# castorini/dhr

Measured on AMD Instinct MI355X. Metric: queries/sec (exact top-1000, brute-force dense-hybrid GIP retrieval), higher is better.
Workload: dtype i8 (bound GEMM: gated AND ungated columns int8 x int8 -> int32 on the matrix cores, every gated rounding upward, the ungated quantisation error paid by the filter margin) + f64-accumulated f16 x f32 exact rescoring of the survivors -- the returned scores are the exact scores rounded once, identical

## Files before the change

### dhr_amd/_lib.py

```python
from __future__ import annotations

import ctypes as C
import os

import numpy as np

from . import _build

DHR_OK = 0
ERR_INVALID, ERR_UNSUPPORTED, ERR_HIP, ERR_INTERNAL, ERR_NOMEM, ERR_PEER = -1, -2, -3, -4, -5, -6
ABI_INDEX_DESC, ABI_QUERY_BATCH, ABI_SEARCH_STATS, ABI_FILE_INFO, ABI_HOST_SHARD = 0, 1, 2, 3, 4
IDX_NONE, IDX_U8, IDX_I8, IDX_I16 = 0, 1, 2, 3
VAL_F16, VAL_F32 = 0, 1
MEM_HOST, MEM_DEVICE = 0, 1
LEX_RAW, LEX_DENSIFY, LEX_AGG_FULL, LEX_AGG_SEMI = 0, 1, 2, 3
PARAM_CAND_CAP, PARAM_FIRST_ROWS, PARAM_PROFILE, PARAM_MAX_GROWTH, PARAM_SAMPLE_PERIOD, PARAM_GEMM_VARIANT, PARAM_MAIN_CHUNKS, PARAM_PROGRESSIVE_THR, PARAM_AUX_CUS, PARAM_GEMM_EXCLUSIVE, PARAM_OVERLAP_AUX, PARAM_SAMPLE_SHARE, PARAM_ASYNC_CONTROLLER, PARAM_LIST_STRIDE = 1, 2, 3, 4, 5, 6, 7, 8, 9, 10, 11, 12, 13, 14
OPT_DENSE_I8, OPT_GATED_I8 = 1, 2
COMM_TRANSPORT, COMM_WORLD, COMM_RANK, COMM_DEVICE = 0, 1, 2, 3
INFO_DENSE_I8, INFO_I8_SCALE, INFO_I8_ROW_ERR, INFO_I8_ROW_NORM, INFO_ROW_NORM_MAX, INFO_TILE_BYTES, INFO_GATED_I8, INFO_GEMM_KERNEL = 1, 2, 3, 4, 5, 6, 7, 8

EXPORTS = ["dhr_version", "dhr_abi_sizes", "dhr_abi_size", "dhr_debug_fail_alloc", "dhr_set_option", "dhr_index_get_info", "dhr_last_error", "dhr_index_create", "dhr_index_destroy", "dhr_index_set_param",
           "dhr_index_device_bytes", "dhr_search", "dhr_score_rows", "dhr_merge_topk", "dhr_merge_topk_host", "dhr_merge_topk_lists", "dhr_merge_topk_lists_host",
           "dhr_get_stats", "dhr_debug_bound_scores", "dhr_debug_query_margins", "dhr_debug_gemm_time", "dhr_debug_seq_to_tile", "dhr_debug_sharded_repairs", "dhr_search_sample_rank", "dhr_search_union_rank", "dhr_search_begin",
           "dhr_search_finish", "dhr_search_mid_ranks", "dhr_search_mid", "dhr_search_pre_ranks", "dhr_search_pre", "dhr_search_begin_rest", "dhr_search_rerank", "dhr_comm_unique_id", "dhr_comm_create", "dhr_comm_wrap", "dhr_comm_create_callback", "dhr_comm_destroy", "dhr_comm_info", "dhr_comm_abort", "dhr_search_sharded", "dhr_search_sharded_local", "dhr_search_sharded_host", "dhr_pq_create", "dhr_pq_destroy", "dhr_pq_device_bytes", "dhr_pq_search", "dhr_pq_adc_scores", "dhr_pq_last_scan", "dhr_index_save", "dhr_index_file_info", "dhr_index_load", "dhr_densify", "dhr_pq_train", "dhr_pq_encode", "dhr_pq_decode", "dhr_pq_train_nbits", "dhr_pq_encode_nbits", "dhr_pq_decode_nbits", "dhr_write_trec", "dhr_format_float", "dhr_lexical_head", "dhr_aggregate", "dhr_gip_scores_workspace", "dhr_gip_scores", "dhr_gip_scores_backward", "dhr_densify_backward", "dhr_lexical_head_train_workspace", "dhr_lexical_head_train", "dhr_lexical_head_backward", "dhr_maxsim_scores", "dhr_maxsim_scores_backward", "dhr_aggregate_train", "dhr_aggregate_backward", "dhr_term_weight_head",
           "dhr_term_weight_head_backward", "dhr_lexical_proj_workspace", "dhr_lexical_proj_head", "dhr_lexical_proj_train_workspace",
           "dhr_lexical_proj_train", "dhr_lexical_proj_backward", "dhr_train_loss_workspace", "dhr_train_loss"]


class DhrError(RuntimeError):

    def __init__(self, msg, status=None):
        super().__init__(msg)
        self.status = status


class IndexDesc(C.Structure):
    _fields_ = [("device", C.c_int32), ("mem_kind", C.c_int32), ("n_rows", C.c_int64), ("d_dlr", C.c_int32),
                ("d_cls", C.c_int32), ("value", C.c_void_p), ("ld_value", C.c_int64), ("index", C.c_void_p),
                ("index_dtype", C.c_int32), ("idx_buckets", C.c_int32), ("ld_index", C.c_int64),
                ("row_offset", C.c_int64)]


class QueryBatch(C.Structure):
    _fields_ = [("n_queries", C.c_int32), ("mem_kind", C.c_int32), ("value", C.c_void_p), ("value_dtype", C.c_int32),
                ("index_dtype", C.c_int32), ("ld_value", C.c_int64), ("index", C.c_void_p), ("ld_index", C.c_int64)]

# ... 166 lines not shown
    lib.dhr_comm_abort.argtypes = [C.c_void_p]
    lib.dhr_comm_abort.restype = None
    lib.dhr_comm_info.argtypes = [C.c_void_p, C.c_int32]
    lib.dhr_search_sharded.argtypes = [C.c_void_p, C.c_void_p, C.POINTER(QueryBatch), C.c_int32, C.c_void_p, C.c_void_p, C.c_int32, C.c_void_p]
    lib.dhr_search_sharded_local.argtypes = [C.POINTER(C.c_void_p), C.c_int32, C.POINTER(QueryBatch), C.c_int32, C.c_void_p, C.c_void_p, C.c_int32, C.c_void_p]
    lib.dhr_pq_create.argtypes = [C.c_int32, C.c_int32, C.c_int64, C.c_int32, C.c_int32, C.c_int32, C.c_void_p, C.c_void_p, C.c_int64, C.POINTER(C.c_void_p)]
    lib.dhr_pq_destroy.argtypes = [C.c_void_p]
    lib.dhr_pq_destroy.restype = None
    lib.dhr_pq_device_bytes.argtypes = [C.c_void_p]
    lib.dhr_pq_device_bytes.restype = C.c_int64
    lib.dhr_pq_search.argtypes = [C.c_void_p, C.POINTER(QueryBatch), C.c_int32, C.c_void_p, C.c_void_p, C.c_int32, C.c_void_p]
    lib.dhr_pq_adc_scores.argtypes = [C.c_void_p, C.POINTER(QueryBatch), C.c_int64, C.c_int64, C.c_void_p, C.c_void_p]
    lib.dhr_pq_last_scan.argtypes = [C.c_void_p, C.POINTER(C.c_double), C.POINTER(C.c_double)]
    lib.dhr_get_stats.argtypes = [C.c_void_p, C.POINTER(SearchStats)]
    lib.dhr_set_option.argtypes = [C.c_int32, C.c_int64]
    lib.dhr_index_get_info.argtypes = [C.c_void_p, C.c_int32, C.POINTER(C.c_double)]
    lib.dhr_debug_bound_scores.argtypes = [C.c_void_p, C.POINTER(QueryBatch), C.c_int64, C.c_int64, C.c_void_p, C.c_void_p]
    lib.dhr_debug_query_margins.argtypes = [C.c_void_p, C.POINTER(QueryBatch), C.c_void_p, C.c_void_p]
    lib.dhr_debug_gemm_time.argtypes = [C.c_void_p, C.POINTER(QueryBatch), C.c_int32, C.POINTER(C.c_double),
                                        C.POINTER(C.c_double), C.c_void_p]
    if hasattr(lib, "dhr_debug_seq_to_tile"):
        lib.dhr_debug_seq_to_tile.argtypes = [C.c_int64, C.c_int32, C.c_int32, C.c_int64, C.c_int64, C.c_int64, C.POINTER(C.c_int64)]
        lib.dhr_debug_seq_to_tile.restype = None
    lib.dhr_search_sample_rank.argtypes = [C.c_void_p, C.c_int32]
    lib.dhr_search_sample_rank.restype = C.c_int32
    lib.dhr_search_union_rank.argtypes = [C.c_void_p, C.c_int32]
    lib.dhr_search_union_rank.restype = C.c_int32
    lib.dhr_search_begin.argtypes = [C.c_void_p, C.POINTER(QueryBatch), C.c_int32, C.c_void_p, C.c_void_p]
    lib.dhr_search_finish.argtypes = [C.c_void_p, C.c_void_p, C.c_void_p, C.c_void_p, C.c_void_p, C.c_int32, C.c_void_p]
    lib.dhr_search_mid_ranks.argtypes = [C.c_void_p, C.c_int32, C.POINTER(C.c_int32), C.POINTER(C.c_int32)]
    lib.dhr_search_mid_ranks.restype = C.c_int32
    lib.dhr_search_mid.argtypes = [C.c_void_p, C.c_void_p, C.c_int32, C.c_void_p, C.c_void_p]
    lib.dhr_search_pre_ranks.argtypes = [C.c_void_p, C.c_int32, C.POINTER(C.c_int32), C.POINTER(C.c_int32)]
    lib.dhr_search_pre_ranks.restype = C.c_int32
    lib.dhr_search_pre.argtypes = [C.c_void_p, C.POINTER(QueryBatch), C.c_int32, C.c_int32, C.c_void_p, C.c_void_p]
    lib.dhr_search_begin_rest.argtypes = [C.c_void_p, C.c_void_p, C.c_void_p, C.c_void_p]
    _lib = lib
    return lib


def check(rc: int, what: str):
    if rc != DHR_OK:
        raise DhrError(f"{what} failed ({rc}): {load().dhr_last_error().decode()}", status=rc)


_NP_IDX = {np.dtype(np.uint8): IDX_U8, np.dtype(np.int8): IDX_I8, np.dtype(np.int16): IDX_I16}
# ... 44 lines not shown
```

### dhr_amd/csrc/api.hip

```cpp
#include "host_stage.h"

extern "C" int dhr_search(dhr_index* ix, const dhr_query_batch* qb, int32_t k, float* out_scores, int64_t* out_rows,
                          int32_t out_mem_kind, void* stream) try {
  dhr::alloc_checkpoint();
  int rc = check_queries(ix, qb);
  if (rc) return rc;
  if (k <= 0) return set_error(DHR_ERR_INVALID, "k must be > 0");
  if (k > (1 << 20)) return set_error(DHR_ERR_UNSUPPORTED, "k > 1048576 is not supported");
  if (!out_scores || !out_rows) return set_error(DHR_ERR_INVALID, "null output pointer");
  if (!DHR_MEM_KIND_OK(out_mem_kind)) return set_error(DHR_ERR_INVALID, "bad out_mem_kind");
  HIP_TRY(hipSetDevice(ix->device));
  hipStream_t s = (hipStream_t)stream;
  const int Q = qb->n_queries;
  ix->pend.valid = false;
  Events evs;
  hipEvent_t ev0, ev1;
  HIP_TRY(evs.add(&ev0)); HIP_TRY(evs.add(&ev1));
  HIP_TRY(hipEventRecord(ev0, s));
  Timer tm{ix->profile != 0, s, {}, {}};
  dhr_search_stats st{};
  st.n_rows = ix->n_rows; st.n_queries = Q; st.k = k;
  Workspace& w = ix->ws;
  Drain drain{ix, s};
  if ((rc = search_core(ix, w, qb, k, 0, tm, st, s)) != DHR_OK) return rc;
// ... 624 lines not shown
  HIP_TRY(launch_gemm_filter(g, s));
  HIP_TRY(hipStreamSynchronize(s));
  return DHR_OK;
} DHR_CATCH_STATUS

extern "C" int dhr_debug_query_margins(dhr_index* ix, const dhr_query_batch* qb, float* out_host, void* stream) try {
  int rc = check_queries(ix, qb);
  if (rc) return rc;
  if (!out_host) return set_error(DHR_ERR_INVALID, "null output pointer");
  HIP_TRY(hipSetDevice(ix->device));
  hipStream_t s = (hipStream_t)stream;
  Workspace& w = ix->ws;
  if ((rc = ensure_ws(ix, w, qb->n_queries, 1, 0)) != DHR_OK) return rc;
  if ((rc = prep_queries(ix, w, qb, s)) != DHR_OK) return rc;
  HIP_TRY(hipMemcpyAsync(out_host, w.margin, (size_t)qb->n_queries * 4, hipMemcpyDeviceToHost, s));
  HIP_TRY(hipStreamSynchronize(s));
  return DHR_OK;
} DHR_CATCH_STATUS

extern "C" void dhr_debug_seq_to_tile(int64_t seq, int32_t map_mode, int32_t period, int64_t head, int64_t perm_mul, int64_t perm_n, int64_t out[2]) try {
  out[0] = seq_to_tile_fast(seq, map_mode, period, head, perm_mul, perm_n, 1.0 / (double)(perm_n > 0 ? perm_n : 1), 1.0 / (double)(period > 1 ? period - 1 : 1));
  out[1] = seq_to_tile(seq, map_mode, period, head, perm_mul, perm_n);
} DHR_CATCH_VOID
extern "C" int dhr_debug_gemm_time(dhr_index* ix, const dhr_query_batch* qb, int32_t iters, double* ms_out, double* flops_out,
                                   void* stream) try {
  int rc = check_queries(ix, qb);
  if (rc) return rc;
  if (iters <= 0 || !ms_out) return set_error(DHR_ERR_INVALID, "bad iters / null pointer");
  HIP_TRY(hipSetDevice(ix->device));
  hipStream_t s = (hipStream_t)stream;
  Workspace& w = ix->ws;
  const bool open = getenv("DHR_GEMM_TIME_OPEN") && atoi(getenv("DHR_GEMM_TIME_OPEN")) != 0 && w.thr_hat && ix->stats.k > 0 && ix->stats.n_queries == qb->n_queries;
  if ((rc = ensure_ws(ix, w, qb->n_queries, open ? (int)ix->stats.k : 1, 0)) != DHR_OK) return rc;
  if ((rc = prep_queries(ix, w, qb, s)) != DHR_OK) return rc;
  if (open) {
    HIP_TRY(hipMemcpyAsync(w.thr, w.thr_hat, (size_t)w.q_pad * 4, hipMemcpyDeviceToDevice, s));
  } else {
    std::vector<float> inf((size_t)w.q_pad, INFINITY);
    HIP_TRY(hipMemcpyAsync(w.thr, inf.data(), (size_t)w.q_pad * 4, hipMemcpyHostToDevice, s));
  }
  const bool opened = open;
  HIP_TRY(hipMemsetAsync(w.cnt, 0, (size_t)w.q_pad * 4, s));
  GemmArgs g{};
  g.a_tiles = ix->tiles; g.b_tiles = w.q_tiles; g.ksteps = ix->ksteps; g.ts = ix->ts; g.td = ix->td; g.ts_q = w.ts_q; g.variant = ix->gemm_variant; g.i8_mul = (ix->dense_i8 || ix->gated_i8) ? w.i8_mul : nullptr; g.g8_shift = ix->gated_i8 ? w.g8_shift : nullptr; g.g8_rsum = ix->g8_rsum; g.seq_lo = 0; g.seq_hi = ix->n_tiles; g.map_mode = 0;
  g.period = 1; g.head = 0; g.n_tiles = ix->n_tiles; g.n_qtiles = w.q_pad / TILE_ROWS; g.n_rows = ix->n_rows;
  g.thr = w.thr; g.cand = w.cand; g.cnt = w.cnt; g.cap = (uint32_t)w.cap; g.n_queries = qb->n_queries;
// ... 96 lines not shown
```

### dhr_amd/csrc/dhr_internal.h

```cpp
#pragma once
#include <hip/hip_runtime.h>
#include <hip/hip_fp16.h>
#include <stdint.h>

#include "../../include/dhr_hip.h"
#include "abi_guard.h"

extern "C" int dhr_set_error_message(int code, const char* msg);
extern "C" int dhr_index_device(const dhr_index* ix);
extern "C" void dhr_internal_index_arena(dhr_index* ix, void*** base, size_t** bytes);
extern "C" int dhr_internal_search_begin_async(dhr_index* ix, const dhr_query_batch* qb, int32_t k, float* out_sample_scores_dev, void* stream);
extern "C" void dhr_internal_search_abort(dhr_index* ix);
extern "C" int dhr_internal_search_pre_async(dhr_index* ix, const dhr_query_batch* qb, int32_t k, int32_t r_local, float* out_scores_dev, void* stream);
extern "C" int dhr_internal_search_begin_rest_async(dhr_index* ix, const float* tau_dev, float* out_sample_scores_dev, void* stream);
extern "C" int dhr_internal_search_mid_async(dhr_index* ix, const float* tau_hat_dev, int32_t r_local, float* out_scores_dev, void* stream);
extern "C" int dhr_internal_search_finish_async(dhr_index* ix, const float* tau_hat_dev, float* out_scores, int64_t* out_rows, int32_t* out_count_dev,
                                                int32_t out_mem_kind, void* stream);

namespace dhr {

constexpr int TILE_ROWS = 256;
constexpr int TILE_K = 64;
constexpr int CHUNK = 8;
constexpr int TILE_HALVES = TILE_ROWS * TILE_K;
// ... 283 lines not shown
hipError_t launch_mark_overflow(const uint32_t* cnt, uint32_t cap, int n_queries, uint32_t* fail_flags, hipStream_t s);
hipError_t launch_verify(const uint64_t* topk_keys, int kp, int k, const float* tau_hat, int n_queries, uint32_t* fail_flags,
                         uint32_t* n_fail, hipStream_t s);
hipError_t launch_gather_queries(const float* q32, const int16_t* q_idx, int k_rm, int d_dlr, const int32_t* ids, int n,
                                 float* out32, int16_t* out_idx, hipStream_t s);
hipError_t launch_scatter_keys(const uint64_t* src, uint64_t* dst, int kp, const int32_t* ids, int n, hipStream_t s);
hipError_t launch_emit_scores(const uint64_t* topk_keys, int kp, int n_queries, int r, float* out, hipStream_t s);
hipError_t launch_make_thr(const float* tau, const float* margin, int n_queries, int q_pad, float* thr, hipStream_t s);
hipError_t launch_raise_thr(float* thr_hat, const float* thr_run, int n_queries, hipStream_t s);
hipError_t launch_flag_tau_above(const float* tau_own, const float* tau_ext, int n_queries, uint32_t* fail_flags, hipStream_t s);
hipError_t launch_raise_thr_rank(float* thr_hat, float* tau_hat, const uint64_t* topk_keys, int kp, int r, const float* margin, int n_queries, hipStream_t s);
hipError_t launch_count_ge(const uint64_t* topk_keys, int kp, int k, const float* tau, const uint32_t* fail_flags, int n_queries,
                           int32_t* out, hipStream_t s);
hipError_t launch_merge_topk(int n_queries, int n_in, const float* in_scores, const int64_t* in_rows, int k_out,
                             float* out_scores, int64_t* out_rows, hipStream_t s);
hipError_t launch_merge_lists(int n_queries, int n_lists, int list_len, const float* in_scores, const int64_t* in_rows, int k_out,
                              float* out_scores, int64_t* out_rows, hipStream_t s, int64_t stride_s = 0, int64_t stride_r = 0);

extern int g_gemm_variant;
extern thread_local int g_last_gemm_kernel;
constexpr int RESCORE_CANDS_PER_WG = 32;
constexpr uint32_t FLAT_GRID_MAX = 1u << 20;
constexpr uint32_t FLAT_GRID_ASYNC = 16384;
constexpr int SELECT_THREADS = 1024;

}
```

### dhr_amd/csrc/kernels.hip

```cpp
#include <algorithm>
#include <cstdlib>
#include <mutex>

#include "dhr_internal.h"
#include "gemm_common.h"
#include <type_traits>

namespace dhr {

typedef short short8 __attribute__((ext_vector_type(8)));

static hipError_t ensure_lds_attr(const void* fn, int bytes, int (&have)[64]) {
  static std::mutex mu;
  int dev = 0;
  (void)hipGetDevice(&dev);
  std::lock_guard<std::mutex> lock(mu);
  if (bytes <= have[dev & 63]) return hipSuccess;
  const hipError_t e = hipFuncSetAttribute(fn, hipFuncAttributeMaxDynamicSharedMemorySize, bytes);
  if (e == hipSuccess) have[dev & 63] = bytes;
  return e;
}

__device__ __forceinline__ float wave_sum(float v) {
#pragma unroll
// ... 688 lines not shown
  part[tid] = s;
  __syncthreads();
  for (int d = 1; d < 1024; d <<= 1) {
    const unsigned long long v = tid >= d ? part[tid - d] : 0ull;
    __syncthreads();
    part[tid] += v;
    __syncthreads();
  }
  unsigned long long run = tid ? part[tid - 1] : 0ull;
  for (int q = lo; q < hi; ++q) {
    uint32_t w = seg(q);
    if (run >= arena_entries) w = 0u;
    else if (run + w > arena_entries) w = (uint32_t)(arena_entries - run);
    ovf_off[q] = (uint32_t)(run < arena_entries ? run : arena_entries);
    ovf_cap[q] = w;
    run += seg(q);
  }
}
hipError_t launch_plan_overflow(const uint32_t* cnt_prev, double rows_ratio, uint32_t cap, uint32_t max_extra, uint32_t arena_entries, int n_queries,
                                uint32_t* ovf_off, uint32_t* ovf_cap, hipStream_t s) {
  hipLaunchKernelGGL(plan_overflow_kernel, dim3(1), dim3(1024), 0, s, cnt_prev, rows_ratio, cap, max_extra, arena_entries, n_queries, ovf_off, ovf_cap);
  return hipGetLastError();
}
__device__ __forceinline__ bool flat_block(const uint32_t* __restrict__ offs, int n_queries, uint32_t b, int& q, uint32_t& blk) {
  if (b >= offs[n_queries]) return false;
  int lo = 0, hi = n_queries;
  while (hi - lo > 1) {
    const int mid = (lo + hi) >> 1;
    if (offs[mid] <= b) lo = mid; else hi = mid;
  }
  q = lo; blk = b - offs[lo];
  return true;
}

template <int SL>
__global__ void __launch_bounds__(256) heavy_build_kernel(const __half* __restrict__ vals_rm, int k_rm,
                                                          const void* __restrict__ idx, int idx_dtype, int64_t n_rows,
                                                          int d_dlr, const uint8_t* __restrict__ map, int n_buckets,
                                                          uint32_t* __restrict__ heavy_key, __half* __restrict__ heavy_val,
                                                          const float* __restrict__ g8_inv_cs, int abs_mode) {
  const int lane = threadIdx.x & 63;
  const int64_t wave0 = (int64_t)blockIdx.x * 4 + (threadIdx.x >> 6);
  const int64_t nwaves = (int64_t)gridDim.x * 4;
  for (int64_t row = wave0; row < n_rows; row += nwaves) {
    constexpr int MAXJ = 64 * SL - 1;
    uint32_t key[SL];
#pragma unroll
    for (int sl = 0; sl < SL; ++sl) {
      const int j = lane + 64 * sl;
      key[sl] = 0u;
      if (j < d_dlr) {
        union { _Float16 h; uint16_t u; } cv; cv.h = (_Float16)__half2float(vals_rm[row * k_rm + j]);
        const uint32_t mag = cv.u & 0x7FFFu;
        if (mag) key[sl] = (mag << 16) | (uint32_t)(MAXJ - j);
      }
    }
// ... 29 lines not shown
hipError_t launch_heavy_build(const __half* vals_rm, int k_rm, const void* idx, int idx_dtype, int64_t n_rows, int d_dlr,
                              const uint8_t* map, int n_buckets, uint32_t* heavy_key, __half* heavy_val, const float* g8_inv_cs, int abs_mode, hipStream_t s) {
  if (n_rows <= 0) return hipSuccess;
  const int64_t blocks = (n_rows + 3) / 4;
  if (d_dlr <= 1024)
    hipLaunchKernelGGL(heavy_build_kernel<16>, dim3((unsigned)(blocks < 16384 ? blocks : 16384)), dim3(256), 0, s, vals_rm, k_rm,
                       idx, idx_dtype, n_rows, d_dlr, map, n_buckets, heavy_key, heavy_val, g8_inv_cs, abs_mode);
  else
    hipLaunchKernelGGL(heavy_build_kernel<64>, dim3((unsigned)(blocks < 16384 ? blocks : 16384)), dim3(256), 0, s, vals_rm, k_rm,
                       idx, idx_dtype, n_rows, d_dlr, map, n_buckets, heavy_key, heavy_val, g8_inv_cs, abs_mode);
  return hipGetLastError();
}

static __device__ __forceinline__ uint4 gather16(const void* p) { return *(const uint4*)p; }
static __device__ __forceinline__ uint2 gather8(const void* p) { return *(const uint2*)p; }
#ifndef REFINE_PREFETCH
#define REFINE_PREFETCH 2
#endif
#ifndef REFINE_L2_PREFETCH
#define REFINE_L2_PREFETCH 0
#endif
#ifndef REFINE_WPE
#define REFINE_WPE 8
#endif
#if REFINE_WPE > 0
#define REFINE_ATTR __attribute__((amdgpu_waves_per_eu(REFINE_WPE)))
#else
#define REFINE_ATTR
#endif
template <bool G8>
__global__ void __launch_bounds__(256) REFINE_ATTR refine_kernel(RefineArgs p) {
  static_assert(REFINE_PER_WG % 64 == 0 && HEAVY_B0 == 20 && HEAVY == 64, "4 lanes x 5 entries, then 4 lanes x 11 entries per candidate; 64 candidates per round");
  extern __shared__ uint32_t qw[];
  constexpr int WSLOTS = REFINE_PER_WG / 4;
  __shared__ uint2 sv_c[REFINE_PER_WG];
  __shared__ uint32_t sv_t[REFINE_PER_WG];
  __shared__ double sv_b[G8 ? REFINE_PER_WG : 1];
  __shared__ uint16_t sv_s[REFINE_PER_WG * 4];
  int q = blockIdx.y;
  uint32_t blk = blockIdx.x;
  const int sub = threadIdx.x & 3, lane = threadIdx.x & 63;
  const uint32_t slot0 = (threadIdx.x >> 6) * WSLOTS;
  for (uint32_t fb = blockIdx.x;; fb += gridDim.x) {
  if (p.blk_off && !flat_block(p.blk_off, p.n_queries, fb, q, blk)) return;
  uint32_t count = p.cnt[q];
  const uint32_t cap_q = p.ovf_cap ? p.cap + p.ovf_cap[q] : p.cap;
  if (count > cap_q) count = cap_q;
  const uint32_t base = blk * REFINE_PER_WG;
  if (base >= count) { if (p.blk_off) continue; return; }
  __syncthreads();
  for (int j = threadIdx.x; j < p.d_dlr; j += 256) {
    if constexpr (G8) { qw[2 * j] = p.q_pack[(int64_t)q * p.d_dlr + j]; qw[2 * j + 1] = p.g8_q8[(int64_t)q * p.d_dlr + j]; }
    else qw[j] = p.q_pack[(int64_t)q * p.d_dlr + j];
  }
  __syncthreads();
  const float t = p.thr[q];
  const double unit = G8 ? (double)p.g8_unit[q] : 0.0;
  const uint32_t end = base + REFINE_PER_WG;
  auto look = [&](const uint32_t key, const uint32_t hbits, int& taken, double& back, float& corr) __attribute__((always_inline)) {
    if (key == 0xFFFFFFFFu) return;
    const uint32_t j = key >> 20;
    union { uint16_t u; _Float16 h; } dv; dv.u = (uint16_t)hbits;
    if constexpr (G8) {
      const uint2 wq = *(const uint2*)(qw + 2 * j);
      const uint32_t w = wq.x;
      const bool same_bucket = p.ungated || ((w >> 12) & 0x1u) == ((key >> 16) & 0x1u);
      const bool mismatch = !p.ungated && (w & 0xFFFu) != (key & 0xFFFu);
      const int lvl = (int)(((key >> 17) & 0x7u) << 4 | ((key >> 12) & 0xFu));
      if (same_bucket && lvl > 0) {
        taken += (int)wq.y * lvl;
        if (!mismatch) {
          union { uint16_t u; _Float16 h; } qv; qv.u = (uint16_t)(w >> 16);
          const float d = p.abs_mode ? fabsf((float)dv.h) : (float)dv.h;
          back += (double)(float)qv.h * (double)d;
        }
      }
    } else {
      const uint32_t w = qw[j];
      const bool same_bucket = ((w >> 12) & 0xFu) == ((key >> 16) & 0xFu);
      const bool mismatch = (w & 0xFFFu) != (key & 0xFFFu);
// ... 6 lines not shown
    float u2 = (float)v;
    if ((double)u2 < v) u2 = nextafterf(u2, INFINITY);
    return u2;
  };
  auto entry = [&](uint32_t i) __attribute__((always_inline)) -> uint2 {
    if (i >= count || i >= end) return make_uint2(0u, 0u);
    return i < p.cap ? p.cand[(int64_t)q * p.cap + i] : p.ovf[(size_t)p.ovf_off[q] + (i - p.cap)];
  };
  struct Rec1 { uint4 a, b; };
  auto record1 = [&](uint32_t i, const uint2 c, Rec1& r) __attribute__((always_inline)) {
    r.a = make_uint4(0xFFFFFFFFu, 0xFFFFFFFFu, 0xFFFFFFFFu, 0xFFFFFFFFu);
    r.b = make_uint4(0xFFFFFFFFu, 0u, 0u, 0u);
    if (i < count && i < end) {
      const uint32_t* h = p.heavy_key + (int64_t)c.x * HEAVY_KEY_STRIDE + sub * 8;
      r.a = gather16(h);
      r.b = gather16(h + 4);
    }
  };
  uint32_t n_w = 0;
  const uint32_t i_first = base + (threadIdx.x >> 2);
#if REFINE_PREFETCH >= 1
  uint2 c_cur = entry(i_first), c_nx = entry(i_first + 64);
#endif
#if REFINE_PREFETCH >= 2
  Rec1 r_cur;
  record1(i_first, c_cur, r_cur);
#endif
  for (uint32_t i = i_first; i < end; i += 64) {
#if REFINE_PREFETCH >= 2
    const uint2 c = c_cur;
    const Rec1 rc = r_cur;
    Rec1 r_nx;
    record1(i + 64, c_nx, r_nx);
    const uint2 c_nx2 = entry(i + 128);
    c_cur = c_nx; c_nx = c_nx2; r_cur = r_nx;
#elif REFINE_PREFETCH == 1
    const uint2 c = c_cur;
    c_cur = c_nx; c_nx = entry(i + 128);
    Rec1 rc;
    record1(i, c, rc);
#else
    const uint2 c = entry(i);
    Rec1 rc;
    record1(i, c, rc);
#endif
    float corr = 0.f;
// ... 11 lines not shown
      taken += __shfl_xor(taken, 1, 64); taken += __shfl_xor(taken, 2, 64);
      back += __shfl_xor(back, 1, 64); back += __shfl_xor(back, 2, 64);
    } else {
      corr += __shfl_xor(corr, 1, 64);
      corr += __shfl_xor(corr, 2, 64);
    }
    bool keep = false;
    if (valid) {
      if constexpr (G8) keep = nextafterf(bound_g8(c.y, taken, back), INFINITY) >= t;
      else keep = __uint_as_float(c.y) - corr >= t;
    }
    const unsigned long long m = __ballot(keep);
    if (keep) {
      const uint32_t slot = slot0 + n_w + (uint32_t)__popcll(m & ((1ull << (lane & ~3)) - 1ull)) / 4u;
      sv_s[slot * 4 + sub] = (uint16_t)(rc.b.w >> 16);
      if (sub == 0) {
        sv_c[slot] = c;
        if constexpr (G8) { sv_t[slot] = (uint32_t)taken; sv_b[slot] = back; }
        else sv_t[slot] = __float_as_uint(corr);
      }
    }
    n_w += (uint32_t)__popcll(m) / 4u;
  }
  __syncthreads();
  n_w = (uint32_t)__builtin_amdgcn_readfirstlane((int)n_w);
  struct Rec2 { uint4 a, b, c, d; };
  auto record2 = [&](uint32_t k, Rec2& r) __attribute__((always_inline)) {
    r.a = r.b = make_uint4(0xFFFFFFFFu, 0xFFFFFFFFu, 0xFFFFFFFFu, 0xFFFFFFFFu);
    r.c = make_uint4(0xFFFFFFFFu, 0xFFFFFFFFu, 0xFFFFFFFFu, 0u);
    r.d = make_uint4(0u, 0u, 0u, 0u);
    if (k < n_w) {
      const uint32_t* h = p.heavy_key + (int64_t)sv_c[slot0 + k].x * HEAVY_KEY_STRIDE + 32 + sub * 16;
      r.a = gather16(h);
      r.b = gather16(h + 4);
      r.c = gather16(h + 8);
      r.d = gather16(h + 12);
    }
  };
#if REFINE_L2_PREFETCH
  Rec2 s_cur;
  record2((uint32_t)(lane >> 2), s_cur);
#endif
  for (uint32_t k0 = 0; k0 < n_w; k0 += 16) {
    const uint32_t k = k0 + (uint32_t)(lane >> 2);
#if REFINE_L2_PREFETCH
    const Rec2 rc = s_cur;
    record2(k + 16, s_cur);
// ... 67 lines not shown
  if (n_rows <= 0) return hipSuccess;
  const int64_t blocks = (n_rows * (resid_ld / 8) + 255) / 256;
  hipLaunchKernelGGL(resid_build_kernel, dim3((unsigned)(blocks < 65536 ? blocks : 65536)), dim3(256), 0, s, vals_rm, k_rm, n_rows, d_dlr, d_cls, col_scale, resid8, resid_ld);
  return hipGetLastError();
}
#ifndef DENSE_REFINE_WPE
#define DENSE_REFINE_WPE 8
#endif
#if DENSE_REFINE_WPE > 0
#define DENSE_REFINE_ATTR __attribute__((amdgpu_waves_per_eu(DENSE_REFINE_WPE)))
#else
#define DENSE_REFINE_ATTR
#endif
#ifndef DENSE_REFINE_LPC
#define DENSE_REFINE_LPC 16
#endif
template <int CH>
__global__ void __launch_bounds__(256) DENSE_REFINE_ATTR dense_refine_kernel(RefineArgs p) {
  constexpr int LPC = DENSE_REFINE_LPC, PB = 128 / LPC, WPP = PB / 4;
  static_assert(LPC == 16 || LPC == 8, "one load instruction of a candidate's lanes = one 128-byte line");
  __shared__ float a_s[1024];
  __shared__ uint32_t f_s[2 * 128];
  __shared__ float red[3 * 4];
  int q = blockIdx.y;
  uint32_t blk = blockIdx.x;
  const int sub = threadIdx.x & (LPC - 1), lane = threadIdx.x & 63, wave = threadIdx.x >> 6;
  constexpr int NCOL = CH * 16;
  for (uint32_t fb = blockIdx.x;; fb += gridDim.x) {
  if (p.blk_off && !flat_block(p.blk_off, p.n_queries, fb, q, blk)) return;
  uint32_t count = p.cnt[q];
  const uint32_t cap_q = p.ovf_cap ? p.cap + p.ovf_cap[q] : p.cap;
  if (count > cap_q) count = cap_q;
  const uint32_t base = blk * REFINE_PER_WG;
  if (base >= count) { if (p.blk_off) continue; return; }
  __syncthreads();
  float mx = 0.f;
  for (int j = threadIdx.x; j < NCOL; j += 256) {
    const float a = j < p.d_cls ? p.q32[(int64_t)q * p.q32_ld + j] * p.col_scale[j] * (1.f / 14.f) : 0.f;
    a_s[j] = a;
    mx = fmaxf(mx, fabsf(a));
  }
#pragma unroll
  for (int o = 32; o > 0; o >>= 1) mx = fmaxf(mx, __shfl_xor(mx, o, 64));
  if (lane == 0) red[wave] = mx;
  __syncthreads();
  mx = fmaxf(fmaxf(red[0], red[1]), fmaxf(red[2], red[3]));
  const float sa = mx > 0.f && mx < INFINITY ? mx * (1.f / 127.f) : 1.f, inv_sa = 1.f / sa;
  float s8 = 0.f, sd = 0.f;
  for (int g8 = threadIdx.x; g8 < NCOL / 8; g8 += 256) {
    uint32_t fe = 0u, fo = 0u;
#pragma unroll
    for (int e = 0; e < 8; ++e) {
      const float a = a_s[g8 * 8 + e];
      float r = rintf(a * inv_sa);
      r = r < -127.f ? -127.f : (r > 127.f ? 127.f : r);
      s8 += r;
      sd += fabsf(a - sa * r);
      const uint32_t b = (uint32_t)(int)r & 0xffu;
      if (e & 1) fo |= b << (8 * (e >> 1)); else fe |= b << (8 * (e >> 1));
    }
    f_s[g8] = fe;
    f_s[128 + g8] = fo;
  }
  s8 = wave_sum(s8); sd = wave_sum(sd);
  if (lane == 0) { red[4 + wave] = s8; red[8 + wave] = sd; }
  __syncthreads();
  s8 = red[4] + red[5] + red[6] + red[7];
  sd = (red[8] + red[9] + red[10] + red[11]) * 1.0001f;
  constexpr int U = CH / 16;
  uint32_t fe[WPP * U], fo[WPP * U];
#pragma unroll
  for (int u = 0; u < U; ++u)
#pragma unroll
    for (int h = 0; h < WPP; ++h) { fe[WPP * u + h] = f_s[32 * u + WPP * sub + h]; fo[WPP * u + h] = f_s[128 + 32 * u + WPP * sub + h]; }
  const int off = 8 * (int)s8;
  const float t = p.thr[q] + p.thr_raise[q] - 7.f * sd;
  struct Piece { uint32_t w[WPP]; };
  constexpr int CPR = 256 / LPC;
  auto fetch = [&](uint32_t i, uint2& c, Piece (&v)[U]) __attribute__((always_inline)) {
    c = make_uint2(0u, 0u);
#pragma unroll
    for (int u = 0; u < U; ++u)
#pragma unroll
      for (int h = 0; h < WPP; ++h) v[u].w[h] = 0x88888888u;
    if (i < count) {
      c = i < p.cap ? p.cand[(int64_t)q * p.cap + i] : p.ovf[(size_t)p.ovf_off[q] + (i - p.cap)];
      const uint8_t* r = p.resid8 + (int64_t)c.x * p.resid_ld + sub * PB;
#pragma unroll
      for (int u = 0; u < U; ++u) {
        if constexpr (PB == 8) { const uint2 t = gather8(r + u * 128); v[u].w[0] = t.x; v[u].w[1] = t.y; }
        else { const uint4 t = gather16(r + u * 128); v[u].w[0] = t.x; v[u].w[1] = t.y; v[u].w[WPP - 2] = t.z; v[u].w[WPP - 1] = t.w; }
      }
    }
  };
  uint2 c;
  Piece v[U];
  fetch(base + (threadIdx.x / LPC), c, v);
  for (uint32_t i = base + (threadIdx.x / LPC); i < base + REFINE_PER_WG; i += CPR) {
    uint2 cn;
// ... 5 lines not shown
#pragma unroll
      for (int h = 0; h < WPP; ++h) {
        isum = __builtin_amdgcn_sdot4((int)fe[WPP * u + h], (int)(v[u].w[h] & 0x0f0f0f0fu), isum, false);
        isum = __builtin_amdgcn_sdot4((int)fo[WPP * u + h], (int)((v[u].w[h] >> 4) & 0x0f0f0f0fu), isum, false);
      }
    }
#pragma unroll
    for (int o = 1; o < LPC; o <<= 1) isum += __shfl_xor(isum, o, 64);
    if (sub == 0 && i < count) {
      float u2 = __uint_as_float(c.y) + sa * (float)(isum - off);
      u2 += fabsf(u2) * 4.8e-7f;
      if (u2 >= t) {
        const uint32_t slot = atomicAdd(p.out_cnt + q, 1u);
        if (slot < p.out_cap) p.out[(int64_t)q * p.out_cap + slot] = make_uint2(c.x, __float_as_uint(u2));
      }
    }
    c = cn;
#pragma unroll
    for (int u = 0; u < U; ++u) v[u] = vn[u];
  }
  if (!p.blk_off) return;
  }
}
hipError_t launch_refine(const RefineArgs& a, hipStream_t s) {
  if (a.max_count == 0 || a.n_queries <= 0) return hipSuccess;
  if (a.resid8) {
    const dim3 grid = a.blk_off ? dim3(std::min<uint32_t>(a.flat_blocks, FLAT_GRID_MAX)) : dim3((a.max_count + REFINE_PER_WG - 1) / REFINE_PER_WG, (unsigned)a.n_queries);
    if (a.blk_off && !a.flat_blocks) return hipSuccess;
    switch (a.resid_ld / 8) {
      case 16: hipLaunchKernelGGL(dense_refine_kernel<16>, grid, dim3(256), 0, s, a); break;
      case 32: hipLaunchKernelGGL(dense_refine_kernel<32>, grid, dim3(256), 0, s, a); break;
      case 48: hipLaunchKernelGGL(dense_refine_kernel<48>, grid, dim3(256), 0, s, a); break;
      case 64: hipLaunchKernelGGL(dense_refine_kernel<64>, grid, dim3(256), 0, s, a); break;
      default: return hipErrorInvalidValue;
    }
    return hipGetLastError();
  }
  const bool g8 = a.g8_q8 != nullptr;
  const size_t lds = (size_t)a.d_dlr * (g8 ? 8 : 4);
  const dim3 grid = a.blk_off ? dim3(std::min<uint32_t>(a.flat_blocks, FLAT_GRID_MAX)) : dim3((a.max_count + REFINE_PER_WG - 1) / REFINE_PER_WG, (unsigned)a.n_queries);
  if (a.blk_off && !a.flat_blocks) return hipSuccess;
  if (g8) hipLaunchKernelGGL(refine_kernel<true>, grid, dim3(256), lds, s, a);
  else hipLaunchKernelGGL(refine_kernel<false>, grid, dim3(256), lds, s, a);
  return hipGetLastError();
}

__device__ __forceinline__ float fmix_lo(uint32_t a, uint32_t b) { float r; asm("v_fma_mix_f32 %0, %1, %2, 0 op_sel_hi:[1,1,0]" : "=v"(r) : "v"(a), "v"(b)); return r; }
__device__ __forceinline__ float fmix_hi(uint32_t a, uint32_t b) { float r; asm("v_fma_mix_f32 %0, %1, %2, 0 op_sel:[1,1,0] op_sel_hi:[1,1,0]" : "=v"(r) : "v"(a), "v"(b)); return r; }
typedef unsigned short ushort2v __attribute__((ext_vector_type(2)));
__device__ __forceinline__ uint32_t pair_mask(uint32_t x, uint32_t sel) {
  union { uint32_t u; ushort2v v; } t, one;
  t.u = __builtin_amdgcn_perm(0u, x, sel);
  one.u = 0x00010001u;
  t.v = __builtin_elementwise_min(t.v, one.v);
  t.v = t.v - one.v;
  return t.u;
}
__device__ __forceinline__ uint32_t pair_mask16(uint32_t x) {
  union { uint32_t u; ushort2v v; } t, one;
  t.u = x;
  one.u = 0x00010001u;
  t.v = __builtin_elementwise_min(t.v, one.v);
  t.v = t.v - one.v;
  return t.u;
}
template <int PATH>
__device__ __forceinline__ void rescore_block(const RescoreArgs& p, const int q, const uint32_t blk) {
  const int lane = threadIdx.x & 63;
  const int wave = threadIdx.x >> 6;
  uint32_t count;
  if (p.cand) { count = p.cnt[q]; if (count > p.cap) count = p.cap; }
  else if (p.rows32) count = p.count_all;
  else count = p.count_all;
  const uint32_t base = blk * RESCORE_CANDS_PER_WG;
  if (base >= count) return;
  const float* q32 = p.q32 + (int64_t)q * p.k_rm;
  const int16_t* qi = p.q_idx + (int64_t)q * p.d_dlr;
  const int nchunks = p.k_rm >> 3;
  const int dlr_chunks = p.d_dlr >> 3;
  const bool fast = p.q16 && *p.q_inexact == 0u && (!p.gate || p.d_dlr == 0 || p.c_idx_dtype == DHR_IDX_U8 || p.c_idx_dtype == DHR_IDX_I8);
  const bool some_zero = p.q_inexact && p.q_inexact[1] != 0u;
  uint32_t nz_mask = some_zero ? 0u : 0xFFFFFFFFu;
  for (int c = lane, t = 0; some_zero && c < nchunks; c += 64, ++t) {
    const float4 qa = *(const float4*)(q32 + c * 8);
    const float4 qb = *(const float4*)(q32 + c * 8 + 4);
    if (qa.x != 0.f || qa.y != 0.f || qa.z != 0.f || qa.w != 0.f || qb.x != 0.f || qb.y != 0.f || qb.z != 0.f || qb.w != 0.f) nz_mask |= 1u << t;
  }
// ... 1160 lines not shown
```

### include/dhr_hip.h

```cpp
#ifndef DHR_HIP_H
#define DHR_HIP_H

#include <stdint.h>

#ifdef __cplusplus
extern "C" {
#endif

#define DHR_VERSION 105

typedef enum dhr_status {
  DHR_OK = 0,
  DHR_ERR_INVALID = -1,
  DHR_ERR_UNSUPPORTED = -2,
  DHR_ERR_HIP = -3,
  DHR_ERR_INTERNAL = -4,
  DHR_ERR_NOMEM = -5,
  DHR_ERR_PEER = -6
} dhr_status;

typedef enum dhr_idx_dtype { DHR_IDX_NONE = 0, DHR_IDX_U8 = 1, DHR_IDX_I8 = 2, DHR_IDX_I16 = 3 } dhr_idx_dtype;
typedef enum dhr_val_dtype { DHR_VAL_F16 = 0, DHR_VAL_F32 = 1 } dhr_val_dtype;
typedef enum dhr_mem_kind { DHR_MEM_HOST = 0, DHR_MEM_DEVICE = 1 } dhr_mem_kind;

// ... 216 lines not shown
                  const float* codebooks, uint8_t* codes, void* stream);
int dhr_pq_decode(int32_t device, int32_t mem_kind, const uint8_t* codes, int64_t n, int32_t d, int32_t M, const float* codebooks,
                  void* out_values_f16, int64_t ld_out, void* stream);
int dhr_pq_train_nbits(int32_t device, int32_t mem_kind, const void* values_f16, int64_t ld, int64_t n, int32_t d, int32_t M, int32_t nbits,
                       int32_t iters, int64_t max_points, float* codebooks, double* out_error, void* stream);
int dhr_pq_encode_nbits(int32_t device, int32_t mem_kind, const void* values_f16, int64_t ld, int64_t n, int32_t d, int32_t M, int32_t nbits,
                        const float* codebooks, uint8_t* codes, void* stream);
int dhr_pq_decode_nbits(int32_t device, int32_t mem_kind, const uint8_t* codes, int64_t n, int32_t d, int32_t M, int32_t nbits,
                        const float* codebooks, void* out_values_f16, int64_t ld_out, void* stream);

int dhr_write_trec(const char* path, int32_t append, int64_t n_queries, int64_t k, const char* qid_blob, const int64_t* qid_off,
                   const char* docid_blob, const int64_t* docid_off, int64_t n_docs, const int64_t* rows, int64_t row_base,
                   const float* scores, const char* run_name, int32_t id_sep_bytes, int32_t n_threads, int64_t* lines_out);
int dhr_format_float(double x, char* out, int32_t cap);

int dhr_get_stats(const dhr_index* index, dhr_search_stats* out);

int dhr_debug_bound_scores(dhr_index* index, const dhr_query_batch* queries, int64_t row_lo, int64_t row_hi,
                           float* out_dev, void* stream);

int dhr_debug_query_margins(dhr_index* index, const dhr_query_batch* queries, float* out_host, void* stream);

void dhr_debug_seq_to_tile(int64_t seq, int32_t map_mode, int32_t period, int64_t head, int64_t perm_mul, int64_t perm_n, int64_t out[2]);
int64_t dhr_debug_fail_alloc(int64_t n);
int32_t dhr_debug_sharded_repairs(void);

int dhr_debug_gemm_time(dhr_index* index, const dhr_query_batch* queries, int32_t iters, double* ms_out,
                        double* flops_out, void* stream);

typedef struct dhr_pq dhr_pq;
int dhr_pq_create(int32_t device, int32_t mem_kind, int64_t n, int32_t d, int32_t M, int32_t nbits, const float* codebooks,
                  const uint8_t* codes, int64_t row_offset, dhr_pq** out);
void dhr_pq_destroy(dhr_pq* pq);
int64_t dhr_pq_device_bytes(const dhr_pq* pq);
int dhr_pq_search(dhr_pq* pq, const dhr_query_batch* queries, int32_t k, float* out_scores, int64_t* out_rows, int32_t out_mem_kind,
                  void* stream);
int dhr_pq_adc_scores(dhr_pq* pq, const dhr_query_batch* queries, int64_t row_lo, int64_t row_hi, float* out_dev, void* stream);
int dhr_pq_last_scan(const dhr_pq* pq, double* ms, double* code_bytes);

typedef struct dhr_comm dhr_comm;
int dhr_comm_unique_id(void* out128, int32_t out_bytes);
int dhr_comm_create(const void* unique_id128, int32_t world, int32_t rank, int32_t device, dhr_comm** out);
int dhr_comm_wrap(void* nccl_comm, int32_t world, int32_t rank, int32_t device, dhr_comm** out);
typedef int (*dhr_allgather_fn)(void* user, const void* send, void* recv, int64_t bytes);
int dhr_comm_create_callback(int32_t world, int32_t rank, int32_t device, dhr_allgather_fn allgather, void* user, dhr_comm** out);
void dhr_comm_destroy(dhr_comm* comm);
// ... 30 lines not shown
```

Baseline: 61620.

## Assign contiguous block runs per workgroup in refine kernels and reuse query staging

The refine kernels previously used a grid-stride loop with a binary search per flat block and restaged query weights on every block. Each workgroup now walks a contiguous range of flat blocks, with a default run of four blocks per workgroup and a floor on grid size. It restages query data and thresholds only when the query changes, and the middle full-workgroup barrier is replaced by a wavefront-level fence. The aim is to cut per-block search and LDS staging overhead, at the cost of a smaller grid and possible load imbalance. The wave-level fence is only safe if that section never shares LDS across waves.

```diff
diff --git a/dhr_amd/_lib.py b/dhr_amd/_lib.py
--- a/dhr_amd/_lib.py
+++ b/dhr_amd/_lib.py
@@ -21,7 +21,7 @@
 
 EXPORTS = ["dhr_version", "dhr_abi_sizes", "dhr_abi_size", "dhr_debug_fail_alloc", "dhr_set_option", "dhr_index_get_info", "dhr_last_error", "dhr_index_create", "dhr_index_destroy", "dhr_index_set_param",
            "dhr_index_device_bytes", "dhr_search", "dhr_score_rows", "dhr_merge_topk", "dhr_merge_topk_host", "dhr_merge_topk_lists", "dhr_merge_topk_lists_host",
-           "dhr_get_stats", "dhr_debug_bound_scores", "dhr_debug_query_margins", "dhr_debug_gemm_time", "dhr_debug_seq_to_tile", "dhr_debug_sharded_repairs", "dhr_search_sample_rank", "dhr_search_union_rank", "dhr_search_begin",
+           "dhr_get_stats", "dhr_debug_bound_scores", "dhr_debug_query_margins", "dhr_debug_gemm_time", "dhr_debug_seq_to_tile", "dhr_debug_block_walk", "dhr_debug_sharded_repairs", "dhr_search_sample_rank", "dhr_search_union_rank", "dhr_search_begin",
            "dhr_search_finish", "dhr_search_mid_ranks", "dhr_search_mid", "dhr_search_pre_ranks", "dhr_search_pre", "dhr_search_begin_rest", "dhr_search_rerank", "dhr_comm_unique_id", "dhr_comm_create", "dhr_comm_wrap", "dhr_comm_create_callback", "dhr_comm_destroy", "dhr_comm_info", "dhr_comm_abort", "dhr_search_sharded", "dhr_search_sharded_local", "dhr_search_sharded_host", "dhr_pq_create", "dhr_pq_destroy", "dhr_pq_device_bytes", "dhr_pq_search", "dhr_pq_adc_scores", "dhr_pq_last_scan", "dhr_index_save", "dhr_index_file_info", "dhr_index_load", "dhr_densify", "dhr_pq_train", "dhr_pq_encode", "dhr_pq_decode", "dhr_pq_train_nbits", "dhr_pq_encode_nbits", "dhr_pq_decode_nbits", "dhr_write_trec", "dhr_format_float", "dhr_lexical_head", "dhr_aggregate", "dhr_gip_scores_workspace", "dhr_gip_scores", "dhr_gip_scores_backward", "dhr_densify_backward", "dhr_lexical_head_train_workspace", "dhr_lexical_head_train", "dhr_lexical_head_backward", "dhr_maxsim_scores", "dhr_maxsim_scores_backward", "dhr_aggregate_train", "dhr_aggregate_backward", "dhr_term_weight_head",
            "dhr_term_weight_head_backward", "dhr_lexical_proj_workspace", "dhr_lexical_proj_head", "dhr_lexical_proj_train_workspace",
            "dhr_lexical_proj_train", "dhr_lexical_proj_backward", "dhr_train_loss_workspace", "dhr_train_loss"]
@@ -234,6 +234,9 @@
     if hasattr(lib, "dhr_debug_seq_to_tile"):
         lib.dhr_debug_seq_to_tile.argtypes = [C.c_int64, C.c_int32, C.c_int32, C.c_int64, C.c_int64, C.c_int64, C.POINTER(C.c_int64)]
         lib.dhr_debug_seq_to_tile.restype = None
+    if hasattr(lib, "dhr_debug_block_walk"):
+        lib.dhr_debug_block_walk.argtypes = [C.c_void_p, C.c_int32, C.c_uint32, C.c_uint32, C.c_void_p, C.c_void_p, C.c_int64]
+        lib.dhr_debug_block_walk.restype = C.c_int64
     lib.dhr_search_sample_rank.argtypes = [C.c_void_p, C.c_int32]
     lib.dhr_search_sample_rank.restype = C.c_int32
     lib.dhr_search_union_rank.argtypes = [C.c_void_p, C.c_int32]
diff --git a/dhr_amd/csrc/api.hip b/dhr_amd/csrc/api.hip
--- a/dhr_amd/csrc/api.hip
+++ b/dhr_amd/csrc/api.hip
@@ -670,6 +670,19 @@
   out[0] = seq_to_tile_fast(seq, map_mode, period, head, perm_mul, perm_n, 1.0 / (double)(perm_n > 0 ? perm_n : 1), 1.0 / (double)(period > 1 ? period - 1 : 1));
   out[1] = seq_to_tile(seq, map_mode, period, head, perm_mul, perm_n);
 } DHR_CATCH_VOID
+extern "C" int64_t dhr_debug_block_walk(const uint32_t* offs, int32_t n_queries, uint32_t n_wg, uint32_t wg, int32_t* out_q, uint32_t* out_blk,
+                                        int64_t max_out) try {
+  if (!offs || n_queries <= 0) return 0;
+  BlockWalk w;
+  if (!block_walk_begin(offs, n_queries, n_wg, wg, w)) return 0;
+  int64_t n = 0;
+  int q; uint32_t blk;
+  while (block_walk_next(offs, w, q, blk)) {
+    if (n < max_out) { if (out_q) out_q[n] = q; if (out_blk) out_blk[n] = blk; }
+    ++n;
+  }
+  return n;
+} DHR_CATCH_VALUE(0)
 extern "C" int dhr_debug_gemm_time(dhr_index* ix, const dhr_query_batch* qb, int32_t iters, double* ms_out, double* flops_out,
                                    void* stream) try {
   int rc = check_queries(ix, qb);
diff --git a/dhr_amd/csrc/dhr_internal.h b/dhr_amd/csrc/dhr_internal.h
--- a/dhr_amd/csrc/dhr_internal.h
+++ b/dhr_amd/csrc/dhr_internal.h
@@ -329,6 +329,51 @@
 constexpr int RESCORE_CANDS_PER_WG = 32;
 constexpr uint32_t FLAT_GRID_MAX = 1u << 20;
 constexpr uint32_t FLAT_GRID_ASYNC = 16384;
+constexpr uint32_t FLAT_GRID_FLOOR = 2048;
 constexpr int SELECT_THREADS = 1024;
 
-}
+__host__ __device__ inline uint32_t uniform_word(const uint32_t* p) {
+#if defined(__HIP_DEVICE_COMPILE__)
+  uint32_t v;
+  asm volatile("s_load_dword %0, %1, 0x0\n\ts_waitcnt lgkmcnt(0)" : "=s"(v) : "s"(p));
+  return v;
+#else
+  return *p;
+#endif
+}
+struct BlockWalk {
+  uint32_t b, end;
+  uint32_t q_lo, q_hi;
+  int q;
+};
+__host__ __device__ inline bool block_walk_begin(const uint32_t* __restrict__ offs, int n_queries, uint32_t n_wg, uint32_t wg, BlockWalk& w) {
+  const uint32_t total = offs[n_queries];
+  if (total == 0u || n_wg == 0u) return false;
+  const uint32_t len = (total - 1u) / n_wg + 1u;
+  const uint64_t lo = (uint64_t)wg * len;
+  if (lo >= total) return false;
+  w.b = (uint32_t)lo;
+  w.end = lo + len < total ? (uint32_t)(lo + len) : total;
+  int a = 0, z = n_queries;
+  while (z - a > 1) {
+    const int mid = (a + z) >> 1;
+    if (offs[mid] <= w.b) a = mid; else z = mid;
+  }
+  w.q = a; w.q_lo = offs[a]; w.q_hi = offs[a + 1];
+  return true;
+}
+__host__ __device__ inline bool block_walk_next(const uint32_t* __restrict__ offs, BlockWalk& w, int& q, uint32_t& blk) {
+  if (w.b >= w.end) return false;
+  while (w.b >= w.q_hi) { ++w.q; w.q_lo = w.q_hi; w.q_hi = uniform_word(offs + w.q + 1); }
+  q = w.q; blk = w.b - w.q_lo;
+  ++w.b;
+  return true;
+}
+inline uint32_t flat_grid(uint32_t blocks, uint32_t run) {
+  if (blocks <= FLAT_GRID_FLOOR || blocks == FLAT_GRID_ASYNC || run <= 1u) return blocks < FLAT_GRID_MAX ? blocks : FLAT_GRID_MAX;
+  uint32_t g = (blocks - 1u) / run + 1u;
+  if (g < FLAT_GRID_FLOOR) g = FLAT_GRID_FLOOR;
+  return g < FLAT_GRID_MAX ? g : FLAT_GRID_MAX;
+}
+
+}
diff --git a/dhr_amd/csrc/kernels.hip b/dhr_amd/csrc/kernels.hip
--- a/dhr_amd/csrc/kernels.hip
+++ b/dhr_amd/csrc/kernels.hip
@@ -734,16 +734,6 @@
   hipLaunchKernelGGL(plan_overflow_kernel, dim3(1), dim3(1024), 0, s, cnt_prev, rows_ratio, cap, max_extra, arena_entries, n_queries, ovf_off, ovf_cap);
   return hipGetLastError();
 }
-__device__ __forceinline__ bool flat_block(const uint32_t* __restrict__ offs, int n_queries, uint32_t b, int& q, uint32_t& blk) {
-  if (b >= offs[n_queries]) return false;
-  int lo = 0, hi = n_queries;
-  while (hi - lo > 1) {
-    const int mid = (lo + hi) >> 1;
-    if (offs[mid] <= b) lo = mid; else hi = mid;
-  }
-  q = lo; blk = b - offs[lo];
-  return true;
-}
 
 template <int SL>
 __global__ void __launch_bounds__(256) heavy_build_kernel(const __half* __restrict__ vals_rm, int k_rm,
@@ -819,6 +809,9 @@
 #endif
 #ifndef REFINE_WPE
 #define REFINE_WPE 8
+#endif
+#ifndef REFINE_MID_BARRIER
+#define REFINE_MID_BARRIER 0
 #endif
 #if REFINE_WPE > 0
 #define REFINE_ATTR __attribute__((amdgpu_waves_per_eu(REFINE_WPE)))
@@ -834,25 +827,24 @@
   __shared__ uint32_t sv_t[REFINE_PER_WG];
   __shared__ double sv_b[G8 ? REFINE_PER_WG : 1];
   __shared__ uint16_t sv_s[REFINE_PER_WG * 4];
-  int q = blockIdx.y;
+  int q = blockIdx.y, q_staged = -1;
   uint32_t blk = blockIdx.x;
   const int sub = threadIdx.x & 3, lane = threadIdx.x & 63;
   const uint32_t slot0 = (threadIdx.x >> 6) * WSLOTS;
-  for (uint32_t fb = blockIdx.x;; fb += gridDim.x) {
-  if (p.blk_off && !flat_block(p.blk_off, p.n_queries, fb, q, blk)) return;
-  uint32_t count = p.cnt[q];
-  const uint32_t cap_q = p.ovf_cap ? p.cap + p.ovf_cap[q] : p.cap;
-  if (count > cap_q) count = cap_q;
+  BlockWalk walk;
+  if (p.blk_off && !block_walk_begin(p.blk_off, p.n_queries, gridDim.x, blockIdx.x, walk)) return;
+  uint32_t count = 0u;
+  float t = 0.f;
+  double unit = 0.0;
+  for (;;) {
+  if (p.blk_off && !block_walk_next(p.blk_off, walk, q, blk)) return;
+  if (q != q_staged) {
+    count = p.cnt[q];
+    const uint32_t cap_q = p.ovf_cap ? p.cap + p.ovf_cap[q] : p.cap;
+    if (count > cap_q) count = cap_q;
+  }
   const uint32_t base = blk * REFINE_PER_WG;
   if (base >= count) { if (p.blk_off) continue; return; }
-  __syncthreads();
-  for (int j = threadIdx.x; j < p.d_dlr; j += 256) {
-    if constexpr (G8) { qw[2 * j] = p.q_pack[(int64_t)q * p.d_dlr + j]; qw[2 * j + 1] = p.g8_q8[(int64_t)q * p.d_dlr + j]; }
-    else qw[j] = p.q_pack[(int64_t)q * p.d_dlr + j];
-  }
-  __syncthreads();
-  const float t = p.thr[q];
-  const double unit = G8 ? (double)p.g8_unit[q] : 0.0;
   const uint32_t end = base + REFINE_PER_WG;
   auto look = [&](const uint32_t key, const uint32_t hbits, int& taken, double& back, float& corr) __attribute__((always_inline)) {
     if (key == 0xFFFFFFFFu) return;
@@ -905,6 +897,17 @@
 #if REFINE_PREFETCH >= 1
   uint2 c_cur = entry(i_first), c_nx = entry(i_first + 64);
 #endif
+  if (q != q_staged) {
+    __syncthreads();
+    for (int j = threadIdx.x; j < p.d_dlr; j += 256) {
+      if constexpr (G8) { qw[2 * j] = p.q_pack[(int64_t)q * p.d_dlr + j]; qw[2 * j + 1] = p.g8_q8[(int64_t)q * p.d_dlr + j]; }
+      else qw[j] = p.q_pack[(int64_t)q * p.d_dlr + j];
+    }
+    t = p.thr[q];
+    if constexpr (G8) unit = (double)p.g8_unit[q];
+    q_staged = q;
+    __syncthreads();
+  }
 #if REFINE_PREFETCH >= 2
   Rec1 r_cur;
   record1(i_first, c_cur, r_cur);
@@ -962,7 +965,13 @@
     }
     n_w += (uint32_t)__popcll(m) / 4u;
   }
-  __syncthreads();
+#if REFINE_MID_BARRIER
+  __syncthreads();
+#else
+  __builtin_amdgcn_fence(__ATOMIC_RELEASE, "wavefront");
+  __builtin_amdgcn_wave_barrier();
+  __builtin_amdgcn_fence(__ATOMIC_ACQUIRE, "wavefront");
+#endif
   n_w = (uint32_t)__builtin_amdgcn_readfirstlane((int)n_w);
   struct Rec2 { uint4 a, b, c, d; };
   auto record2 = [&](uint32_t k, Rec2& r) __attribute__((always_inline)) {
@@ -1076,17 +1085,28 @@
   __shared__ float a_s[1024];
   __shared__ uint32_t f_s[2 * 128];
   __shared__ float red[3 * 4];
-  int q = blockIdx.y;
+  int q = blockIdx.y, q_staged = -1;
   uint32_t blk = blockIdx.x;
   const int sub = threadIdx.x & (LPC - 1), lane = threadIdx.x & 63, wave = threadIdx.x >> 6;
   constexpr int NCOL = CH * 16;
-  for (uint32_t fb = blockIdx.x;; fb += gridDim.x) {
-  if (p.blk_off && !flat_block(p.blk_off, p.n_queries, fb, q, blk)) return;
-  uint32_t count = p.cnt[q];
-  const uint32_t cap_q = p.ovf_cap ? p.cap + p.ovf_cap[q] : p.cap;
-  if (count > cap_q) count = cap_q;
+  constexpr int U = CH / 16;
+  BlockWalk walk;
+  if (p.blk_off && !block_walk_begin(p.blk_off, p.n_queries, gridDim.x, blockIdx.x, walk)) return;
+  uint32_t count = 0u;
+  uint32_t fe[WPP * U], fo[WPP * U];
+  float sa = 1.f, t = 0.f;
+  int off = 0;
+  for (;;) {
+  if (p.blk_off && !block_walk_next(p.blk_off, walk, q, blk)) return;
+  if (q != q_staged) {
+    count = p.cnt[q];
+    const uint32_t cap_q = p.ovf_cap ? p.cap + p.ovf_cap[q] : p.cap;
+    if (count > cap_q) count = cap_q;
+  }
   const uint32_t base = blk * REFINE_PER_WG;
   if (base >= count) { if (p.blk_off) continue; return; }
+  if (q != q_staged) {
+  q_staged = q;
   __syncthreads();
   float mx = 0.f;
   for (int j = threadIdx.x; j < NCOL; j += 256) {
@@ -1099,7 +1119,8 @@
   if (lane == 0) red[wave] = mx;
   __syncthreads();
   mx = fmaxf(fmaxf(red[0], red[1]), fmaxf(red[2], red[3]));
-  const float sa = mx > 0.f && mx < INFINITY ? mx * (1.f / 127.f) : 1.f, inv_sa = 1.f / sa;
+  sa = mx > 0.f && mx < INFINITY ? mx * (1.f / 127.f) : 1.f;
+  const float inv_sa = 1.f / sa;
   float s8 = 0.f, sd = 0.f;
   for (int g8 = threadIdx.x; g8 < NCOL / 8; g8 += 256) {
     uint32_t fe = 0u, fo = 0u;
@@ -1121,14 +1142,13 @@
   __syncthreads();
   s8 = red[4] + red[5] + red[6] + red[7];
   sd = (red[8] + red[9] + red[10] + red[11]) * 1.0001f;
-  constexpr int U = CH / 16;
-  uint32_t fe[WPP * U], fo[WPP * U];
 #pragma unroll
   for (int u = 0; u < U; ++u)
 #pragma unroll
     for (int h = 0; h < WPP; ++h) { fe[WPP * u + h] = f_s[32 * u + WPP * sub + h]; fo[WPP * u + h] = f_s[128 + 32 * u + WPP * sub + h]; }
-  const int off = 8 * (int)s8;
-  const float t = p.thr[q] + p.thr_raise[q] - 7.f * sd;
+  off = 8 * (int)s8;
+  t = p.thr[q] + p.thr_raise[q] - 7.f * sd;
+  }
   struct Piece { uint32_t w[WPP]; };
   constexpr int CPR = 256 / LPC;
   auto fetch = [&](uint32_t i, uint2& c, Piece (&v)[U]) __attribute__((always_inline)) {
@@ -1180,10 +1200,14 @@
   if (!p.blk_off) return;
   }
 }
+static uint32_t refine_run_blocks() {
+  static const uint32_t run = getenv("DHR_REFINE_RUN") ? (uint32_t)std::max(1, atoi(getenv("DHR_REFINE_RUN"))) : 4u;
+  return run;
+}
 hipError_t launch_refine(const RefineArgs& a, hipStream_t s) {
   if (a.max_count == 0 || a.n_queries <= 0) return hipSuccess;
   if (a.resid8) {
-    const dim3 grid = a.blk_off ? dim3(std::min<uint32_t>(a.flat_blocks, FLAT_GRID_MAX)) : dim3((a.max_count + REFINE_PER_WG - 1) / REFINE_PER_WG, (unsigned)a.n_queries);
+    const dim3 grid = a.blk_off ? dim3(flat_grid(a.flat_blocks ? a.flat_blocks : 1u, refine_run_blocks())) : dim3((a.max_count + REFINE_PER_WG - 1) / REFINE_PER_WG, (unsigned)a.n_queries);
     if (a.blk_off && !a.flat_blocks) return hipSuccess;
     switch (a.resid_ld / 8) {
       case 16: hipLaunchKernelGGL(dense_refine_kernel<16>, grid, dim3(256), 0, s, a); break;
@@ -1196,7 +1220,7 @@
   }
   const bool g8 = a.g8_q8 != nullptr;
   const size_t lds = (size_t)a.d_dlr * (g8 ? 8 : 4);
-  const dim3 grid = a.blk_off ? dim3(std::min<uint32_t>(a.flat_blocks, FLAT_GRID_MAX)) : dim3((a.max_count + REFINE_PER_WG - 1) / REFINE_PER_WG, (unsigned)a.n_queries);
+  const dim3 grid = a.blk_off ? dim3(flat_grid(a.flat_blocks ? a.flat_blocks : 1u, refine_run_blocks())) : dim3((a.max_count + REFINE_PER_WG - 1) / REFINE_PER_WG, (unsigned)a.n_queries);
   if (a.blk_off && !a.flat_blocks) return hipSuccess;
   if (g8) hipLaunchKernelGGL(refine_kernel<true>, grid, dim3(256), lds, s, a);
   else hipLaunchKernelGGL(refine_kernel<false>, grid, dim3(256), lds, s, a);
@@ -1221,6 +1245,16 @@
   t.v = __builtin_elementwise_min(t.v, one.v);
   t.v = t.v - one.v;
   return t.u;
+}
+__device__ __forceinline__ bool flat_block(const uint32_t* __restrict__ offs, int n_queries, uint32_t b, int& q, uint32_t& blk) {
+  if (b >= offs[n_queries]) return false;
+  int lo = 0, hi = n_queries;
+  while (hi - lo > 1) {
+    const int mid = (lo + hi) >> 1;
+    if (offs[mid] <= b) lo = mid; else hi = mid;
+  }
+  q = lo; blk = b - offs[lo];
+  return true;
 }
 template <int PATH>
 __device__ __forceinline__ void rescore_block(const RescoreArgs& p, const int q, const uint32_t blk) {
diff --git a/include/dhr_hip.h b/include/dhr_hip.h
--- a/include/dhr_hip.h
+++ b/include/dhr_hip.h
@@ -262,6 +262,7 @@
 int dhr_debug_query_margins(dhr_index* index, const dhr_query_batch* queries, float* out_host, void* stream);
 
 void dhr_debug_seq_to_tile(int64_t seq, int32_t map_mode, int32_t period, int64_t head, int64_t perm_mul, int64_t perm_n, int64_t out[2]);
+int64_t dhr_debug_block_walk(const uint32_t* offs, int32_t n_queries, uint32_t n_wg, uint32_t wg, int32_t* out_q, uint32_t* out_blk, int64_t max_out);
 int64_t dhr_debug_fail_alloc(int64_t n);
 int32_t dhr_debug_sharded_repairs(void);
 
```

After: 61730, median of 2. No clear change (+0.2%).
